# fani-lab/OpeNTF

Hardware: AMD Instinct MI355X
Metric: teams/sec (train) bnn_emb d=128 on DBLP (higher is better)
Workload: dtype f32 (fp16x3 split products, f32 accumulate)

## Files before the change

### opentf_amd/csrc/ntf_engine.hip

```cpp
#include "../../include/opentf_amd.h"
#include "ntf_kernels.h"
#include "ntf_fused.h"
#include "ntf_head.h"

#include <algorithm>
#include <cmath>
#include <cstdio>
#include <cstdlib>
#include <cstring>
#include <string>
#include <vector>

using namespace ntf;

static thread_local std::string g_create_error;

struct LayerInfo {
    int in = 0, out = 0;
    int64_t off[4] = {0, 0, 0, 0};
    int64_t nw() const { return (int64_t)in * out; }
};

enum Fam { F_GATHER = 0, F_GEMM_HIDDEN, F_FLIPOUT_OPERAND, F_OUT_FWD, F_LOSS, F_OUT_BWD_DW, F_OUT_BWD_DA, F_BIAS_GRAD,
           F_FLIPOUT_FINAL, F_KL, F_ADAM, F_SAMPLER, F_INFER, F_OUT_FUSED_FWD, F_OUT_FUSED_DW, F_OUT_FUSED_AUX, F_MULTIHOT, F_COUNT };
// ... 46 lines not shown
    float *partial = nullptr, *row_fix = nullptr, *d_loss = nullptr, *ent_mc = nullptr, *ent_mean = nullptr;
    float *dh_slab = nullptr;
    char* fws = nullptr;
    char* fws_set[2] = {nullptr, nullptr};
    int head_prefetch = 1;
    struct { bool valid = false; uint64_t step = 0; const int64_t* rows = nullptr; int B = 0; int ub = -1; } hp;
    const int64_t* hp_next_rows = nullptr; int hp_next_B = 0;
    const int64_t* hp_next_host = nullptr;
    bool hidden_adam_done = false;
    int64_t hp_used = 0;
    float* gemm_slab = nullptr;
    double* d_kl = nullptr; double* d_acc = nullptr; int64_t* d_acc_steps = nullptr;
    int fwd_kernel = -1;
    int lean = 1;
    int dw_ksplit = 0;
    int32_t* d_range = nullptr;
    int64_t range_fallbacks_host = 0;
    float* tk_vals = nullptr; int32_t* tk_idx = nullptr; int64_t tk_cap = 0;
    std::vector<float*> inj_eps_w, inj_eps_b, inj_s_in, inj_s_out;
    uint64_t seed = 0, step = 0;
    int maxhid = 0;
    int timing = 0;
    std::vector<TimeRec> recs;
    std::vector<hipEvent_t> pool;
    double fam_ms[F_COUNT] = {0}; int64_t fam_calls[F_COUNT] = {0};
    int last_global_B = 0; int last_B = 0; float last_dz_packed_scale = 0.f;
    bool adam_in_dw = false;
    int f32_copy_merged = 1;
    uint64_t f32_copy_step = 0;
    int merge_bias = 1;
// ... 107 lines not shown
    if (cfg->mfma < 0 || cfg->mfma > NTF_MFMA_FP16X3) { g_create_error = "bad mfma"; return NTF_EINVAL; }
    if (cfg->input_mode == NTF_INPUT_MULTIHOT && cfg->n_layers < 2) { g_create_error = "multi-hot input needs a hidden layer (src/mdl/fnn.py:17-19)"; return NTF_EINVAL; }
    int ndev = 0;
    if (hipGetDeviceCount(&ndev) != hipSuccess || ndev < 1) { g_create_error = "no HIP device: the engine has no CPU fallback"; return NTF_EHIP; }
    if (cfg->device < 0 || cfg->device >= ndev) { g_create_error = "device ordinal out of range"; return NTF_EINVAL; }
    if (hipSetDevice(cfg->device) != hipSuccess) { g_create_error = "hipSetDevice failed"; return NTF_EHIP; }
    ntf_engine* e = new ntf_engine();
    e->cfg = *cfg;
    e->L = cfg->n_layers;
    e->lr = cfg->lr;
    e->seed = cfg->seed;
    if (const char* fk = getenv("NTF_FWD_KERNEL")) {
        e->fwd_kernel = atoi(fk);
        if (e->fwd_kernel != 0 && e->fwd_kernel != 5) { g_create_error = "NTF_FWD_KERNEL: 5 (k_out_fwd_h3p, the default) or 0 (k_out_fwd_b6); the forms 1-4 of rounds 2-3 are retired"; delete e; return NTF_EINVAL; }
    }
    if (const char* ks = getenv("NTF_DW_KSPLIT")) e->dw_ksplit = atoi(ks);
    if (const char* ln = getenv("NTF_LEAN")) e->lean = atoi(ln);
    if (const char* hp = getenv("NTF_HEAD_PREFETCH")) e->head_prefetch = atoi(hp);
    if (const char* pf = getenv("NTF_PREFETCH")) e->prefetch = atoi(pf);
    if (const char* hd = getenv("NTF_HEAD")) e->head = atoi(hd);
    if (const char* mb = getenv("NTF_MERGE_BIAS")) e->merge_bias = atoi(mb);
    if (const char* sw = getenv("NTF_L0_SWEEP")) e->l0_sweep = atoi(sw);
    if (const char* fp = getenv("NTF_FNN_PIPE")) e->fnn_pipe = atoi(fp);
    if (const char* mh = getenv("NTF_MH_HEAD")) e->mh_head = atoi(mh);
    if (const char* ek = getenv("NTF_EVAL_KERNEL")) e->eval_kernel = atoi(ek);
    if (const char* nf = getenv("NTF_INFER_F32")) e->infer_f32 = atoi(nf);
    if (const char* fc = getenv("NTF_F32_COPY_MERGED")) e->f32_copy_merged = atoi(fc);
    if (const char* eh = getenv("NTF_EP_HEAD_PREFETCH")) e->ep_head_prefetch = atoi(eh);
    if (const char* dr = getenv("NTF_DP_RANGES")) e->dp_ranges = atoi(dr);
    if (const char* ds = getenv("NTF_DP_SIDE_BWD")) e->dp_side_bwd = atoi(ds);
    if (const char* sb = getenv("NTF_SIDE_BWD")) e->side_bwd = atoi(sb);
// ... 812 lines not shown
        if (side && l == e->L - 2) e->st = e->st3;
        const float* in = e->act[l];
        float* gW = e->G + li.off[NTF_P_WEIGHT]; float* gb = e->G + li.off[NTF_P_BIAS];
        float* gRW = e->cfg.bayesian ? e->G + li.off[NTF_P_RHO_WEIGHT] : nullptr;
        float* gRb = e->cfg.bayesian ? e->G + li.off[NTF_P_RHO_BIAS] : nullptr;
        SignSpec sin_, sout_;
        if (e->cfg.bayesian) { sin_ = sign_spec(e, c, l, T_S_IN, li.in); sout_ = sign_spec(e, c, l, T_S_OUT, li.out); }
        if (last && fused) {
            FusedDw f;
            f.B = B; f.H = li.in; f.M = M; f.bayes = e->cfg.bayesian;
            f.dzT = e->dZout; f.h = in; f.g_mu = gW; f.g_rho = gRW; f.g_b = gb; f.g_bp = gRb; f.ws = e->fws;
            f.mu = e->P + li.off[NTF_P_WEIGHT];
            f.s_out = sout_; f.s_out_inj = e->cfg.bayesian && (sout_.inj != nullptr || sin_.inj != nullptr);
            f.split = e->cfg.mfma != NTF_MFMA_F32 && split_products(e);
            f.a_scale = dz_scale16(e, c.global_B); f.h_scale = kH16Scale; f.rflag = range_ptr(e);
            f.dz_packed = f.split && li.in == 128 && e->pl_mu != nullptr;
            e->last_dz_packed_scale = f.dz_packed ? f.a_scale : 0.f;
            if (f.dz_packed && !c.defer_dw && !(c.fuse_adam && e->cfg.fuse_adam == 2)) {
                const int tiles = (M + fused_dw_tile() - 1) / fused_dw_tile(), nib = fused_ldb(B) / 32;
                int ks = e->dw_ksplit > 0 ? e->dw_ksplit : (tiles <= 128 ? std::min({256 / tiles, 8, std::max(1, nib / 4)}) : 1);
                while (ks > 1 && fused_dw_part_floats(M, li.in, ks) > (int64_t)e->cfg.max_batch * M) --ks;
                if (ks > 1) { f.ksplit = ks; f.part = e->Zout; }
            }
            if (e->cfg.bayesian) { f.rho = e->P + li.off[NTF_P_RHO_WEIGHT]; f.wp = e->Wp[l]; f.klw = kl_share / ((float)out_nw * (float)c.global_B); f.cur_eps = normal_spec(e, c, l, T_EPS_W); }
            if (c.defer_dw) {
                const int tile = fused_dw_tile(), total = (M + tile - 1) / tile;
                e->pend = f; e->pend_valid = true; e->pend_chunks = (total + 255) / 256;
                if (e->cfg.bayesian) { e->pend_eps_b = normal_spec(e, c, l, T_EPS_B); e->pend_klw_b = kl_share / ((float)out_nb * (float)c.global_B); }
                continue;
            }
// ... 54 lines not shown
                    if (gRW) HIPCHK(e, hipMemsetAsync(gRW, 0, (size_t)li.nw() * 4, e->st));
                }
                e->g0_clean = false; e->pre0_step = ~0ull;
                if (l0_sweep_now) HIPCHK(e, hipMemsetAsync(e->l0_touched, 0, (size_t)li.in, e->st));
                launch_multihot_bwd(e->st, c.rows_dev, B, li.in, li.out, e->s_indptr, e->s_indices, dZ, sin_, sout_, gW, gRW, l0_sweep_now ? e->l0_touched : nullptr);
            } else {
                Scope t(e, last ? F_OUT_BWD_DW : F_GEMM_HIDDEN);
                GemmArgs g;
                g.M = li.out; g.N = li.in; g.K = B;
                g.A = dZ; g.sam = 1; g.sak = li.out;
                g.B = in; g.sbk = li.in; g.sbn = 1;
                g.C = gW; g.ldc = li.in;
                const int wtiles = ((li.out + 63) / 64) * ((li.in + 63) / 64);
                if (wtiles < 64 && B >= 256) { g.ksplit = std::max(1, std::min({B >= 2048 ? 64 : 16, B / 64, (int)(kGemmSlabFloats / ((int64_t)li.out * li.in))})); g.slab = e->gemm_slab; }
                if (g.ksplit <= 1) { g.ksplit = 1; g.slab = nullptr; }
                launch_gemm(e->st, g);
                if (e->cfg.bayesian) { g.sa = sout_; g.sa_t = 1; g.sb = sin_; g.sb_t = 0; g.C = gRW; launch_gemm(e->st, g); }
            }
            if (l > 0) {
                Scope t(e, last ? F_OUT_BWD_DA : F_GEMM_HIDDEN);
                float* dA = e->dAct[l & 1];
                GemmArgs g;
                g.M = B; g.N = li.in; g.K = li.out;
                g.A = dZ; g.sam = li.out; g.sak = 1;
                g.B = e->P + li.off[NTF_P_WEIGHT]; g.sbk = li.in; g.sbn = 1;
                g.C = dA; g.ldc = li.in;
                g.mask = e->act[l]; g.ldmask = li.in;
                const int tiles = ((B + 63) / 64) * ((li.in + 63) / 64);
                int ks = 1;
                if (li.out >= 4096) ks = std::max(1, std::min({64, 1024 / tiles, (int)(kGemmSlabFloats / ((int64_t)B * li.in))}));
                g.ksplit = ks; g.slab = e->gemm_slab;
                launch_gemm(e->st, g);
// ... 683 lines not shown
```

### opentf_amd/csrc/ntf_fused.h

```cpp
#pragma once
#include "ntf_kernels.h"

namespace ntf {

struct FusedOut {
    int B = 0, H = 0, M = 0, bayes = 0, train = 0;
    const float* h = nullptr;
    const float *mu = nullptr, *mu_b = nullptr;
    const float *wp = nullptr, *bp = nullptr;
    SignSpec s_in, s_out;
    float tnw = 1.f, tpw = 1.f, inv_B = 1.f;
    float* dzT = nullptr;
    float* dh_slab = nullptr;
    float* dh = nullptr;
    const float* h_mask = nullptr;
    float* loss_partial = nullptr;
    void* ws = nullptr;
    const int64_t* rows = nullptr; const int64_t* m_indptr = nullptr; const int32_t* m_indices = nullptr;
    const int64_t* neg = nullptr; int ns = 0; float* row_fix = nullptr;
    int c_lo = 0;
    int split = 0; uint16_t* mu_pl = nullptr; uint16_t* wp_pl = nullptr;
    float w_scale = 1.f, h_scale = 1.f, dz_scale = 1.f;
    int wide = 5;
    int eval_kernel = 1;
// ... 8 lines not shown

struct FusedDw {
    int B = 0, H = 0, M = 0, bayes = 0;
    const float* dzT = nullptr; const float* h = nullptr;
    const float *mu = nullptr, *rho = nullptr, *wp = nullptr;
    float *g_mu = nullptr, *g_rho = nullptr, *g_b = nullptr, *g_bp = nullptr;
    float klw = 0.f;
    void* ws = nullptr;
    SignSpec s_out; int s_out_inj = 0;
    int adam = 0;
    int split = 0;
    float a_scale = 1.f, h_scale = 1.f;
    int wg_begin = 0, wg_count = 0;
    int* rflag = nullptr;
    int dz_packed = 0;
    int ksplit = 1; float* part = nullptr;
    float *w_mu = nullptr, *w_rho = nullptr, *m_mu = nullptr, *v_mu = nullptr, *m_rho = nullptr, *v_rho = nullptr;
    float lr_over_bc1 = 0.f, b1 = 0.9f, b2 = 0.999f, eps = 1e-8f, bc2_sqrt = 1.f;
    NormalSpec cur_eps;
    int lean = 0;
    int produce = 0; NormalSpec nx_eps; float* nx_wp = nullptr; uint16_t *nx_pl_wp = nullptr, *nx_pl_mu = nullptr; float nx_pscale = 1.f; double nx_klw = 0.0;
    double* nx_kl = nullptr; int* nx_rflag = nullptr;
};

bool fused_supported(int H);
int fused_loss_slots(int M);
int64_t fused_dh_slab_floats(int B, int H, int M);
size_t fused_workspace_bytes(int B, int H, int M);
struct FusedWsPtrs { float *hz, *hs; uint32_t* sinbits; uint16_t* hb; uint32_t* sinT; int Bpad; };
FusedWsPtrs fused_ws_ptrs(void* ws, int B, int H, int M);
// ... 12 lines not shown
```

### opentf_amd/csrc/ntf_fused_dw.hip

```cpp
#include "ntf_fused_common.h"

namespace ntf {

struct DwArgs {
    int B, M, Bpad;
    const float *__restrict__ dzT, *__restrict__ h, *__restrict__ hs, *__restrict__ mu, *__restrict__ rho;
    const float* wp;
    const uint32_t* sbits; int nCB; uint32_t so_k0, so_k1; int so_inj;
    float *__restrict__ g_mu, *__restrict__ g_rho, *__restrict__ g_b, *__restrict__ g_bp;
    float klw;
    float *__restrict__ w_mu, *__restrict__ w_rho, *__restrict__ m_mu, *__restrict__ v_mu, *__restrict__ m_rho, *__restrict__ v_rho;
    float lr_over_bc1, b1, b2, eps, bc2_sqrt;
    int wg_begin;
    int* rflag; int rmode;
    const uint32_t* sT;
    const uint32_t* sinT;
    const uint16_t* hb;
    float a_scale, unscale;
    int ksplit; float* part; int64_t slab; int part_row0;
    unsigned long long* stamps;
    int ntile, stagger;
    NormalSpec cur_eps; int lean;
    int produce; NormalSpec nx_eps; float* nx_wp; uint16_t *nx_pl_wp, *nx_pl_mu; float nx_pscale; double nx_klw; double* nx_kl; int* nx_rflag;
};

__device__ __forceinline__ float adam_update(float p, float g, float& m, float& v, float lr_over_bc1, float b1, float b2, float eps, float bc2_sqrt) {
    adam_step(p, g, m, v, lr_over_bc1, b1, b2, eps, __builtin_amdgcn_rcpf(bc2_sqrt));
    return p;
}

__device__ __forceinline__ uint32_t transpose32(uint32_t a, int il) {
    uint32_t m = 0x0000FFFFu;
#pragma unroll
    for (int j = 16; j != 0; j >>= 1) {
        const uint32_t pv = (uint32_t)__shfl_xor((int)a, j, 64);
// ... 502 lines not shown
#define DWQ_PPG 3
#endif
constexpr int QW = 4;
constexpr int QTC = 32 * QW;
template <bool BAYES, bool ADAM, bool STAMP = false, bool SPLIT = false>
__global__ __launch_bounds__(64 * QW, 2) void k_out_dw_q(DwArgs p) {
    extern __shared__ __attribute__((aligned(16))) char smem[];
    constexpr int H = 128, NJT = 4;
    constexpr int TA = QTC * 32 * 4;
    constexpr int PLANE = H * 64;
    constexpr int TB = 2 * PLANE;
    constexpr int SRC_TB = (BAYES ? 2 : 1) * TB;
    constexpr int TW = BAYES ? 1024 : 0;
    constexpr int STAGE = TA + TB + TW;
    typedef _Float16 h2_t __attribute__((ext_vector_type(2)));
    const int tid = threadIdx.x, lane = tid & 63, wave = tid >> 6, il = lane & 31, half = lane >> 5;
    if (p.rmode == 1 && __builtin_nontemporal_load(p.rflag) != 0) return;
    const int ntile_s = SPLIT ? (int)gridDim.x / p.ksplit : 0;
    const int ksi = SPLIT ? (int)blockIdx.x / ntile_s : 0;
    const int c0 = (p.wg_begin + (SPLIT ? (int)blockIdx.x % ntile_s : (int)blockIdx.x)) * QTC;
    const int crow = wave * 32 + il, c = c0 + crow;
    const int nib = p.Bpad / 32;
    const int ib0 = SPLIT ? (int)((int64_t)ksi * nib / p.ksplit) : 0, ib1 = SPLIT ? (int)((int64_t)(ksi + 1) * nib / p.ksplit) : nib;
    const uint32_t smem_base = lds_addr(smem);
    const int wave_u = __builtin_amdgcn_readfirstlane(wave);
    const char* hb = reinterpret_cast<const char*>(p.hb);
    unsigned long long st_t[4] = {0, 0, 0, 0};
    if (STAMP) st_t[0] = __builtin_amdgcn_s_memrealtime();
    uint32_t lds_base = 0u;
    if (STAMP || (p.stagger > 0 && (int)blockIdx.x < p.ntile)) asm volatile("s_getreg_b32 %0, hwreg(HW_REG_LDS_ALLOC, 0, 8)" : "=s"(lds_base));
    if (p.stagger > 0 && (int)blockIdx.x < p.ntile) {
        if (lds_base != 0u) {
            const uint64_t t0 = __builtin_amdgcn_s_memrealtime();
            while (__builtin_amdgcn_s_memrealtime() - t0 < (uint64_t)p.stagger) __builtin_amdgcn_s_sleep(64);
        }
    }

    const h2_t ones = {(_Float16)1.0f, (_Float16)1.0f};
    constexpr int NA = TA / 1024 / QW, NB = TB / 1024 / QW;
    const float* dz_tile = p.dzT + (int64_t)(c0 >> 8) * nib * 8192 + ((c0 & 255) << 5);
    const uint32_t* sw_src = BAYES ? (half == 0 ? p.sT + (int64_t)(c0 >> 8) * nib * 256 + (c0 & 255) + il * 4 : p.sinT + il * 4) : nullptr;
    const int sw_step = half == 0 ? 256 : 128;
    auto stage_piece = [&](int ib, int buf, int n) {
        const uint32_t sb = smem_base + buf * STAGE;
        if (n < NA) {
            const int inst = wave_u * NA + n;
            const int row = inst * 8 + (lane >> 3), pch = lane & 7;
            const int q = pch ^ ((row >> 1) & 7);
            glds16(dz_tile + (int64_t)ib * 8192 + row * 32 + 4 * q, sb + inst * 1024);
        } else {
            const char* src = hb + (size_t)ib * SRC_TB;
            const int inst = wave_u * NB + (n - NA);
            const int pos = inst * 1024 + lane * 16;
            const int j = (pos % PLANE) >> 6, cd = (pos >> 4) & 3;
            glds16(src + (pos & ~63) + 16 * (cd ^ ((j >> 2) & 3)), sb + TA + inst * 1024);
            if (BAYES && n == NA + NB - 1) glds16(sw_src + (int64_t)ib * sw_step, sb + TA + TB);
        }
    };
    float nx_kl = 0.f, nx_amax = 0.f;
    unsigned long long st_c[3] = {0, 0, 0}, c_prev = 0;
    auto cyc = [&]() -> unsigned long long {
        unsigned long long t;
        __builtin_amdgcn_sched_barrier(0);
        asm volatile("s_memtime %0\n\ts_waitcnt lgkmcnt(0)" : "=s"(t) :: "memory");
        __builtin_amdgcn_sched_barrier(0);
        return t;
    };
#pragma unroll
    for (int n = 0; n < NA + NB; ++n) stage_piece(ib0, 0, n);
    f32x16 acc1[NJT], acc2[NJT];
#pragma unroll
    for (int j = 0; j < NJT; ++j)
#pragma unroll
        for (int r = 0; r < 16; ++r) { acc1[j][r] = 0.f; acc2[j][r] = 0.f; }
    float sum1 = 0.f, sum2 = 0.f;
    const int shl0 = 12 - 4 * half, shl1 = 4 - 4 * half;
    asm volatile("s_waitcnt vmcnt(0)" ::: "memory");
    __syncthreads();
    auto k_block = [&](int ib, auto more_c) {
        constexpr bool MORE = decltype(more_c)::value;
        const int buf = (ib - ib0) & 1;
        const char* sA = smem + buf * STAGE;
        const char* sB = sA + TA;
        uint32_t word = 0u;
        u32x4 iw = {0u, 0u, 0u, 0u};
        if (BAYES) { word = *reinterpret_cast<const uint32_t*>(sA + TA + TB + crow * 4); iw = *reinterpret_cast<const u32x4*>(sA + TA + TB + 512 + il * 16); }
        constexpr int NG = 2 * NJT;
        const char* bbase = sB + il * 64;
        const int swz = (il >> 2) & 3;
        auto load_b = [&](int g, u32x4 (&dst)[2]) {
            const int ks = g / NJT, jt = g % NJT;
            const char* bp = bbase + jt * 2048 + 16 * ((2 * ks + half) ^ swz);
#pragma unroll
// ... 18 lines not shown
                    as[ks][0][q] = s1; as[ks][1][q] = s2;
                    sum2 = __builtin_amdgcn_fdot2(__builtin_bit_cast(h2_t, s1), ones, sum2, false);
                    sum2 = __builtin_amdgcn_fdot2(__builtin_bit_cast(h2_t, s2), ones, sum2, false);
                }
            }
        };
        constexpr int BR = DWQ_BRING;
        u32x4 bq[BR][2], bs[2];
#pragma unroll
        for (int g = 0; g < BR - 1; ++g) load_b(g, bq[g]);
        prep_a(0);
        int piece = 0;
        auto dma = [&]() {
            if (MORE) {
#pragma unroll
                for (int q = 0; q < DWQ_PPG; ++q) { if (piece < NA + NB) stage_piece(ib + 1, buf ^ 1, piece); ++piece; }
            }
        };
#pragma unroll
        for (int g = 0; g < NG; ++g) {
            if (g + BR - 1 < NG) load_b(g + BR - 1, bq[(g + BR - 1) % BR]);
            asm volatile("" ::: "memory");
            const int ks = g / NJT, jt = g % NJT;
            acc1[jt] = mfma3h(a[ks], bq[g % BR], acc1[jt]);
            dma();
            if (BAYES) {
                const uint32_t v = iw[jt] << (ks ? shl1 : shl0);
#pragma unroll
                for (int q = 0; q < 4; ++q) {
                    const uint32_t m = (v << q) & 0x80008000u;
                    bs[0][q] = bq[g % BR][0][q] ^ m; bs[1][q] = bq[g % BR][1][q] ^ m;
                }
                acc2[jt] = mfma3h(as[ks], bs, acc2[jt]);
                dma();
            }
            if (g == 0) prep_a(1);
        }
        if (STAMP) { st_c[0] += cyc() - c_prev; c_prev = cyc(); }
        asm volatile("s_waitcnt vmcnt(0)" ::: "memory");
        if (STAMP) { st_c[1] += cyc() - c_prev; c_prev = cyc(); }
        __syncthreads();
        if (STAMP) { st_c[2] += cyc() - c_prev; c_prev = cyc(); }
    };
    if (STAMP) { st_t[1] = __builtin_amdgcn_s_memrealtime(); c_prev = cyc(); }
    if (DWQ_PRIO) __builtin_amdgcn_s_setprio(DWQ_PRIO);
    for (int ib = ib0; ib < ib1 - 1; ++ib) k_block(ib, std::true_type{});
    k_block(ib1 - 1, std::false_type{});
    if (DWQ_PRIO) __builtin_amdgcn_s_setprio(0);
    if (STAMP) st_t[2] = __builtin_amdgcn_s_memrealtime();
    sum1 += __shfl_xor(sum1, 32, 64);
    sum2 += __shfl_xor(sum2, 32, 64);
    const float inv_a = 1.f / p.a_scale;
    if constexpr (SPLIT) {
        if (half == 0 && c < p.M) {
            float* pb = p.part + (int64_t)p.ksplit * 2 * p.slab; const int64_t Mp = p.slab / 128; const int cl = c - p.part_row0;
            pb[(int64_t)(ksi * 2) * Mp + cl] = sum1 * inv_a; if (BAYES) pb[(int64_t)(ksi * 2 + 1) * Mp + cl] = sum2 * inv_a;
        }
#pragma unroll
        for (int r = 0; r < 16; ++r) {
            const int cr = c0 + wave * 32 + rowmap(r, half);
            if (cr >= p.M) continue;
            const int64_t il0 = (int64_t)(cr - p.part_row0) * H + NJT * il;
            float s1[NJT], s2[NJT];
#pragma unroll
            for (int jt = 0; jt < NJT; ++jt) { s1[jt] = acc1[jt][r] * p.unscale; s2[jt] = acc2[jt][r] * p.unscale; }
            st_vec<NJT>(p.part + (int64_t)(ksi * 2) * p.slab + il0, s1);
            if (BAYES) st_vec<NJT>(p.part + (int64_t)(ksi * 2 + 1) * p.slab + il0, s2);
        }
        return;
    }
    if (half == 0 && c < p.M) { p.g_b[c] = sum1 * inv_a; if (BAYES) p.g_bp[c] = sum2 * inv_a; }

    constexpr int PD = DW_EPI_PD;
    DwOps<NJT> ops[PD + 1];
    auto row_idx = [&](int r, int64_t& idx0) -> bool {
        const int cr = c0 + wave * 32 + rowmap(r, half);
        idx0 = (int64_t)cr * H + NJT * il;
        return cr < p.M;
    };
    static_for<0, PD>([&](auto rc) { constexpr int r = decltype(rc)::value; int64_t idx0; if (row_idx(r, idx0)) dw_ops_load<BAYES, ADAM, NJT>(p, idx0, ops[r % (PD + 1)]); });
    static_for<0, 16>([&](auto rc) {
        constexpr int r = decltype(rc)::value;
        if constexpr (r + PD < 16) { int64_t idn; if (row_idx(r + PD, idn)) dw_ops_load<BAYES, ADAM, NJT>(p, idn, ops[(r + PD) % (PD + 1)]); }
        int64_t idx0;
        if (row_idx(r, idx0)) {
            float s1[NJT], s2[NJT];
#pragma unroll
            for (int jt = 0; jt < NJT; ++jt) { s1[jt] = acc1[jt][r] * p.unscale; s2[jt] = acc2[jt][r] * p.unscale; }
            dw_finish_ops<BAYES, ADAM, NJT>(p, idx0, s1, s2, ops[r % (PD + 1)], nx_kl, nx_amax);
        }
    });
    if (STAMP && p.stamps && lane == 0) {
        asm volatile("s_waitcnt vmcnt(0)" ::: "memory");
        st_t[3] = __builtin_amdgcn_s_memrealtime();
        uint32_t hw_id, xcc;
        asm volatile("s_getreg_b32 %0, hwreg(HW_REG_HW_ID)" : "=s"(hw_id));
        asm volatile("s_getreg_b32 %0, hwreg(HW_REG_XCC_ID)" : "=s"(xcc));
        unsigned long long* o = p.stamps + ((int64_t)blockIdx.x * QW + wave) * 10;
        o[0] = st_t[0]; o[1] = st_t[1]; o[2] = st_t[2]; o[3] = st_t[3]; o[4] = ((unsigned long long)xcc << 32) | hw_id; o[5] = lds_base;
        o[6] = st_c[0]; o[7] = st_c[1]; o[8] = st_c[2]; o[9] = 0;
    }
    if (ADAM && p.produce) dw_produce_finish<BAYES>(p, nx_kl, nx_amax, reinterpret_cast<double*>(smem + 2 * STAGE), QW);
}

void launch_fused_out_dw(hipStream_t st, const FusedDw& f) {
    const Geom g = geom(f.B, f.M);
    const WsLayout w = ws_layout(f.B, f.H, f.M);
    char* ws = static_cast<char*>(f.ws);
    DwArgs a;
    a.B = f.B; a.M = f.M; a.Bpad = g.Bpad; a.dzT = f.dzT; a.h = reinterpret_cast<const float*>(ws + w.hz); a.hs = reinterpret_cast<const float*>(ws + w.hs);
    a.mu = f.mu; a.rho = f.rho; a.wp = f.wp; a.sbits = reinterpret_cast<const uint32_t*>(ws + w.sbits); a.nCB = g.nCB;
    a.so_k0 = f.s_out.k0; a.so_k1 = f.s_out.k1; a.so_inj = f.s_out_inj;
    a.g_mu = f.g_mu; a.g_rho = f.g_rho; a.g_b = f.g_b; a.g_bp = f.g_bp; a.klw = f.klw;
    a.w_mu = f.w_mu; a.w_rho = f.w_rho; a.m_mu = f.m_mu; a.v_mu = f.v_mu; a.m_rho = f.m_rho; a.v_rho = f.v_rho;
    a.lr_over_bc1 = f.lr_over_bc1; a.b1 = f.b1; a.b2 = f.b2; a.eps = f.eps; a.bc2_sqrt = f.bc2_sqrt;
    const int total = (f.M + DW_TC - 1) / DW_TC;
    const int grid = f.wg_count > 0 ? std::min(f.wg_count, total - f.wg_begin) : total;
    a.wg_begin = f.wg_count > 0 ? f.wg_begin : 0;
    if (grid <= 0) return;
    a.hb = reinterpret_cast<const uint16_t*>(ws + w.hb);
    a.rflag = f.rflag; a.rmode = 0;
    a.produce = (f.produce && f.adam && f.H == 128) ? 1 : 0;
    a.cur_eps = f.cur_eps; a.lean = (a.produce && f.lean) ? 1 : 0;
    a.nx_eps = f.nx_eps; a.nx_wp = f.nx_wp; a.nx_pl_wp = f.nx_pl_wp; a.nx_pl_mu = f.nx_pl_mu; a.nx_pscale = f.nx_pscale; a.nx_klw = f.nx_klw; a.nx_kl = f.nx_kl; a.nx_rflag = f.nx_rflag;
    a.ntile = 0; a.stagger = 0; a.stamps = nullptr;
    const bool guard = f.split && f.rflag != nullptr;
    a.sT = reinterpret_cast<const uint32_t*>(ws + w.sbitsT);
    a.ksplit = 1; a.part = nullptr; a.slab = 0; a.part_row0 = 0;
    if (f.H == 256) {
        const size_t lds = 2 * ((size_t)DW_TC * 32 * 4 + (size_t)(f.bayes ? 2 : 1) * 32 * 4 * 128);
#define NTF_DWH(BY, AD) do { auto kf = k_out_dw_h2<BY, AD>; set_max_lds(reinterpret_cast<const void*>(kf), (int)lds);              \
        hipLaunchKernelGGL(kf, dim3(grid, 2), dim3(64 * DW_WAVES), lds, st, a); } while (0)
        if (f.bayes) { if (f.adam) NTF_DWH(true, true); else NTF_DWH(true, false); } else { if (f.adam) NTF_DWH(false, true); else NTF_DWH(false, false); }
#undef NTF_DWH
        return;
    }
    if (f.split && f.dz_packed) {
        a.a_scale = f.a_scale; a.unscale = 1.f / (f.a_scale * f.h_scale); a.rmode = guard ? 1 : 0;
        const int ks = (f.ksplit > 1 && f.part) ? std::min(f.ksplit, std::max(1, g.Bpad / 32)) : 1;
        if (ks > 1) {
// ... 14 lines not shown
            if (!guard) return;
            a.rmode = 2; a.ksplit = 1; a.wg_begin = wg256; a.part_row0 = 0;
            goto exact_f32;
        }
        {
            a.sinT = reinterpret_cast<const uint32_t*>(ws + w.sinT);
            const int total_q = (f.M + QTC - 1) / QTC, qb = f.wg_count > 0 ? 2 * f.wg_begin : 0;
            const int qgrid = f.wg_count > 0 ? std::min(2 * f.wg_count, total_q - qb) : total_q;
            const int wg256 = a.wg_begin;
            a.wg_begin = qb;
            static int n_cu = 0;
            if (!n_cu) { int dev = 0; hipGetDevice(&dev); hipDeviceGetAttribute(&n_cu, hipDeviceAttributeMultiprocessorCount, dev); if (n_cu <= 0) n_cu = 256; }
            static const int stagger_q = getenv("NTF_DW_STAGGER") ? atoi(getenv("NTF_DW_STAGGER")) : -1;
            const int nib = g.Bpad / 32;
            a.ntile = 2 * n_cu;
            a.stagger = (f.adam && qgrid > n_cu) ? (stagger_q >= 0 ? stagger_q : (nib * 140 + 4500) / 2) : 0;
            const size_t ldsq = 2 * ((size_t)QTC * 128 + 2 * 128 * 64 + (f.bayes ? 1024 : 0)) + 64;
#define NTF_DWQ(BY, AD) do { auto kf = k_out_dw_q<BY, AD>;                                                                     \
            set_max_lds(reinterpret_cast<const void*>(kf), (int)ldsq);     \
            hipLaunchKernelGGL(kf, dim3(qgrid), dim3(64 * QW), ldsq, st, a); } while (0)
#ifdef NTF_DIAG
            static const char* stamp_file = getenv("NTF_DW_STAMP_FILE");
#else
            static const char* stamp_file = nullptr;
#endif
            if (stamp_file && f.bayes && f.adam) {
                static unsigned long long* d_st = nullptr; static int n_launch = 0;
                if (!d_st) hipMalloc(&d_st, (size_t)qgrid * QW * 10 * 8);
                a.stamps = d_st;
                auto kf = k_out_dw_q<true, true, true>;
                set_max_lds(reinterpret_cast<const void*>(kf), (int)ldsq);
                hipLaunchKernelGGL(kf, dim3(qgrid), dim3(64 * QW), ldsq, st, a);
                if (++n_launch == 30) {
                    std::vector<unsigned long long> hst((size_t)qgrid * QW * 10);
                    hipStreamSynchronize(st); hipMemcpy(hst.data(), d_st, hst.size() * 8, hipMemcpyDeviceToHost);
                    if (FILE* fp = fopen(stamp_file, "wb")) { fwrite(hst.data(), 8, hst.size(), fp); fclose(fp); }
                }
            }
            else if (f.bayes) { if (f.adam) NTF_DWQ(true, true); else NTF_DWQ(true, false); } else { if (f.adam) NTF_DWQ(false, true); else NTF_DWQ(false, false); }
#undef NTF_DWQ
            if (!guard) return;
            a.rmode = 2; a.wg_begin = wg256; a.ntile = 0; a.stagger = 0;
            goto exact_f32;
        }
    }
    if (f.split) {
        a.rmode = guard ? 1 : 0;
// ... 43 lines not shown
```

### opentf_amd/csrc/ntf_kernels.h

```cpp
#pragma once
#include <hip/hip_runtime.h>
#include <stdint.h>

namespace ntf {

constexpr float kLeakySlope = 0.01f;

struct SignSpec {
    const float* inj = nullptr;
    int64_t ld = 0;
    uint32_t k0 = 0, k1 = 0;
    int enabled = 0;
};

struct NormalSpec {
    const float* inj = nullptr;
    uint32_t k0 = 0, k1 = 0, tag = 0, step = 0;
    int64_t qbase = 0;
};

struct GemmArgs {
    int M = 0, N = 0, K = 0;
    const float* A = nullptr; int64_t sam = 0, sak = 0;
    const float* B = nullptr; int64_t sbk = 0, sbn = 0;
    SignSpec sa; int sa_t = 0;
    SignSpec sb; int sb_t = 0;
    float* C = nullptr; int64_t ldc = 0;
    float* Act = nullptr; int64_t ldact = 0;
    const float* bias = nullptr;
    SignSpec sc;
    const float* mask = nullptr; int64_t ldmask = 0;
    int accumulate = 0;
    int ksplit = 1;
    float* slab = nullptr;
    float alpha = 1.0f;
};

void launch_gemm(hipStream_t st, const GemmArgs& a);

void launch_gather_meanpool(hipStream_t st, const int64_t* indptr, const int32_t* indices, const float* table,
                            const int64_t* rows, int64_t n, int d, int mean, float* out);
void launch_gather_dense_rows(hipStream_t st, const float* X, int d, const int64_t* rows, int64_t n, float* out);
void launch_multihot_fwd(hipStream_t st, const int64_t* rows, int B, int S, int H, const int64_t* indptr, const int32_t* indices,
                         const float* W, const float* b, const float* Wp , const float* bp, SignSpec sin, SignSpec sout, float* act);
void launch_multihot_bwd(hipStream_t st, const int64_t* rows, int B, int S, int H, const int64_t* indptr, const int32_t* indices,
                         const float* dZ, SignSpec sin, SignSpec sout, float* gW , float* gWp , uint8_t* touched = nullptr);

struct PerturbChain { double* kl_out2 = nullptr; int* mu_flag_out = nullptr; const int* raise_if = nullptr; };
void launch_flipout_perturb(hipStream_t st, const float* rho, const float* mu, int64_t n, NormalSpec eps, float* out, double w, double* kl_out,
                            uint16_t* planes_w = nullptr, uint16_t* planes_mu = nullptr, const float* pmu = nullptr, int H = 0,
                            float pscale = 1.f,
                            int* rflag = nullptr ,
                            const int* only_if = nullptr ,
// ... 55 lines not shown
```

### opentf_amd/csrc/ntf_kernels.hip

```cpp
#include "ntf_kernels.h"
#include <cstdlib>
#include "ntf_device.h"
#include <algorithm>
#include <cstdint>

namespace ntf {

constexpr int GBM = 64, GBN = 64, GBK = 32, GLD = GBK + 1;

__global__ __launch_bounds__(256) void k_gemm(GemmArgs a) {
    __shared__ float As[GBM * GLD];
    __shared__ float Bs[GBN * GLD];
    const int tid = threadIdx.x, lane = tid & 63, wave = tid >> 6;
    const int m0 = blockIdx.y * GBM, n0 = blockIdx.x * GBN;
    int kper = (a.K + a.ksplit - 1) / a.ksplit;
    kper = (kper + GBK - 1) / GBK * GBK;
    const int kbeg = blockIdx.z * kper;
    const int kend = min(a.K, kbeg + kper);
    const bool a_kc = (a.sak == 1), b_nc = (a.sbn == 1);
    f32x16 acc;
#pragma unroll
    for (int i = 0; i < 16; ++i) acc[i] = 0.f;
    const int wm = wave >> 1, wn = wave & 1;

// ... 63 lines not shown
    if (e >= mn) return;
    float s = 0.f;
    for (int z = 0; z < ks; ++z) s += slab[(int64_t)z * mn + e];
    const int64_t o = (e / N) * ldc + (e % N);
    C[o] = accumulate ? C[o] + s : s;
}

void launch_gemm(hipStream_t st, const GemmArgs& a) {
    if (a.M <= 0 || a.N <= 0) return;
    dim3 grid((a.N + GBN - 1) / GBN, (a.M + GBM - 1) / GBM, a.ksplit > 1 ? a.ksplit : 1);
    hipLaunchKernelGGL(k_gemm, grid, dim3(256), 0, st, a);
    if (a.ksplit > 1) {
        const int64_t mn = (int64_t)a.M * a.N;
        hipLaunchKernelGGL(k_gemm_reduce, dim3((unsigned)((mn + 255) / 256)), dim3(256), 0, st, a.slab, a.ksplit, mn, a.N, a.C, a.ldc, a.accumulate);
    }
}

template <int G>
__global__ __launch_bounds__(256) void k_gather_pool(const int64_t* __restrict__ indptr, const int32_t* __restrict__ indices,
                                                     const float* __restrict__ table, const int64_t* __restrict__ rows,
                                                     int64_t n, int d, int mean, int vec, float* __restrict__ out) {
    constexpr int TPW = 64 / G;
    const int lane = threadIdx.x & 63, sub = lane / G, sl = lane % G;
    const int64_t wave_global = ((int64_t)blockIdx.x * blockDim.x + threadIdx.x) >> 6;
    const int64_t t = wave_global * TPW + sub;
    const bool live = t < n;
    const int64_t team = live ? (rows ? rows[t] : t) : 0;
    const int64_t beg = live ? indptr[team] : 0, end = live ? indptr[team + 1] : 0;
    const int nnz = (int)(end - beg);
    const int nchunk = (d + 4 * G - 1) / (4 * G);
// ... 904 lines not shown
```

Measured before the change: 676,400.

## Add persistent tile walk to output dW kernel and fused hidden-layer dW kernel

The output-layer dW kernel (k_out_dw_q) can now run as a persistent grid capped at a slot count. Each workgroup walks several column tiles and prefetches the next tile's operands while it runs the current tile's epilogue. A new k_hidden_dw kernel computes the hidden-layer weight gradient and its flipout counterpart in one launch, reducing the k-split partials in LDS instead of going through the slab-plus-reduce GEMM path. This removes launch and reduction-kernel overhead for small hidden layers. The costs are higher register pressure in the persistent loop and a less tiled, f32-MFMA hidden kernel that reads operands straight from global memory.

```diff
diff --git a/opentf_amd/csrc/ntf_engine.hip b/opentf_amd/csrc/ntf_engine.hip
--- a/opentf_amd/csrc/ntf_engine.hip
+++ b/opentf_amd/csrc/ntf_engine.hip
@@ -84,6 +84,9 @@
     int fwd_kernel = -1;
     int lean = 1;
     int dw_ksplit = 0;
+    int dw_persist = 1;
+    int dw_slots = 0;
+    int hidden_dw = 1;
     int32_t* d_range = nullptr;
     int64_t range_fallbacks_host = 0;
     float* tk_vals = nullptr; int32_t* tk_idx = nullptr; int64_t tk_cap = 0;
@@ -221,7 +224,13 @@
         e->fwd_kernel = atoi(fk);
         if (e->fwd_kernel != 0 && e->fwd_kernel != 5) { g_create_error = "NTF_FWD_KERNEL: 5 (k_out_fwd_h3p, the default) or 0 (k_out_fwd_b6); the forms 1-4 of rounds 2-3 are retired"; delete e; return NTF_EINVAL; }
     }
+    if (const char* dk = getenv("NTF_DW_KERNEL")) {
+        if (atoi(dk) != 1) { g_create_error = "NTF_DW_KERNEL: 1 (k_out_dw_q, the default); round 3's one-workgroup-per-CU form 0 was retired in round 6"; delete e; return NTF_EINVAL; }
+    }
     if (const char* ks = getenv("NTF_DW_KSPLIT")) e->dw_ksplit = atoi(ks);
+    if (const char* dp = getenv("NTF_DW_PERSIST")) e->dw_persist = atoi(dp) != 0;
+    if (const char* sl = getenv("NTF_DW_SLOTS")) e->dw_slots = std::max(0, atoi(sl));
+    if (const char* hd = getenv("NTF_HIDDEN_DW")) e->hidden_dw = atoi(hd) != 0;
     if (const char* ln = getenv("NTF_LEAN")) e->lean = atoi(ln);
     if (const char* hp = getenv("NTF_HEAD_PREFETCH")) e->head_prefetch = atoi(hp);
     if (const char* pf = getenv("NTF_PREFETCH")) e->prefetch = atoi(pf);
@@ -1064,6 +1073,7 @@
             f.s_out = sout_; f.s_out_inj = e->cfg.bayesian && (sout_.inj != nullptr || sin_.inj != nullptr);
             f.split = e->cfg.mfma != NTF_MFMA_F32 && split_products(e);
             f.a_scale = dz_scale16(e, c.global_B); f.h_scale = kH16Scale; f.rflag = range_ptr(e);
+            f.persist = e->dw_persist; f.slots = e->dw_slots;
             f.dz_packed = f.split && li.in == 128 && e->pl_mu != nullptr;
             e->last_dz_packed_scale = f.dz_packed ? f.a_scale : 0.f;
             if (f.dz_packed && !c.defer_dw && !(c.fuse_adam && e->cfg.fuse_adam == 2)) {
@@ -1148,8 +1158,14 @@
                 const int wtiles = ((li.out + 63) / 64) * ((li.in + 63) / 64);
                 if (wtiles < 64 && B >= 256) { g.ksplit = std::max(1, std::min({B >= 2048 ? 64 : 16, B / 64, (int)(kGemmSlabFloats / ((int64_t)li.out * li.in))})); g.slab = e->gemm_slab; }
                 if (g.ksplit <= 1) { g.ksplit = 1; g.slab = nullptr; }
+                if (e->hidden_dw && hidden_dw_supported(li.in, li.out)) {
+                    HiddenDw hd; hd.B = B; hd.D = li.in; hd.H = li.out; hd.ksplit = g.ksplit; hd.dz = dZ; hd.x = in; hd.g_w = gW;
+                    if (e->cfg.bayesian) { hd.g_wp = gRW; hd.s_out = sout_; hd.s_in = sin_; }
+                    launch_hidden_dw(e->st, hd);
+                } else {
                 launch_gemm(e->st, g);
                 if (e->cfg.bayesian) { g.sa = sout_; g.sa_t = 1; g.sb = sin_; g.sb_t = 0; g.C = gRW; launch_gemm(e->st, g); }
+                }
             }
             if (l > 0) {
                 Scope t(e, last ? F_OUT_BWD_DA : F_GEMM_HIDDEN);
diff --git a/opentf_amd/csrc/ntf_fused.h b/opentf_amd/csrc/ntf_fused.h
--- a/opentf_amd/csrc/ntf_fused.h
+++ b/opentf_amd/csrc/ntf_fused.h
@@ -46,6 +46,7 @@
     int wg_begin = 0, wg_count = 0;
     int* rflag = nullptr;
     int dz_packed = 0;
+    int persist = 1, slots = 0;
     int ksplit = 1; float* part = nullptr;
     float *w_mu = nullptr, *w_rho = nullptr, *m_mu = nullptr, *v_mu = nullptr, *m_rho = nullptr, *v_rho = nullptr;
     float lr_over_bc1 = 0.f, b1 = 0.9f, b2 = 0.999f, eps = 1e-8f, bc2_sqrt = 1.f;
diff --git a/opentf_amd/csrc/ntf_fused_dw.hip b/opentf_amd/csrc/ntf_fused_dw.hip
--- a/opentf_amd/csrc/ntf_fused_dw.hip
+++ b/opentf_amd/csrc/ntf_fused_dw.hip
@@ -19,6 +19,7 @@
     float a_scale, unscale;
     int ksplit; float* part; int64_t slab; int part_row0;
     unsigned long long* stamps;
+    int nwalk;
     int ntile, stagger;
     NormalSpec cur_eps; int lean;
     int produce; NormalSpec nx_eps; float* nx_wp; uint16_t *nx_pl_wp, *nx_pl_mu; float nx_pscale; double nx_klw; double* nx_kl; int* nx_rflag;
@@ -551,16 +552,17 @@
     constexpr int TW = BAYES ? 1024 : 0;
     constexpr int STAGE = TA + TB + TW;
     typedef _Float16 h2_t __attribute__((ext_vector_type(2)));
-    const int tid = threadIdx.x, lane = tid & 63, wave = tid >> 6, il = lane & 31, half = lane >> 5;
+    int tid = threadIdx.x, lane = tid & 63, wave = tid >> 6, il = lane & 31, half = lane >> 5;
     if (p.rmode == 1 && __builtin_nontemporal_load(p.rflag) != 0) return;
     const int ntile_s = SPLIT ? (int)gridDim.x / p.ksplit : 0;
     const int ksi = SPLIT ? (int)blockIdx.x / ntile_s : 0;
-    const int c0 = (p.wg_begin + (SPLIT ? (int)blockIdx.x % ntile_s : (int)blockIdx.x)) * QTC;
-    const int crow = wave * 32 + il, c = c0 + crow;
+    int t = SPLIT ? (int)blockIdx.x % ntile_s : (int)blockIdx.x;
+    int c0 = (p.wg_begin + t) * QTC;
+    int crow = wave * 32 + il;
     const int nib = p.Bpad / 32;
     const int ib0 = SPLIT ? (int)((int64_t)ksi * nib / p.ksplit) : 0, ib1 = SPLIT ? (int)((int64_t)(ksi + 1) * nib / p.ksplit) : nib;
     const uint32_t smem_base = lds_addr(smem);
-    const int wave_u = __builtin_amdgcn_readfirstlane(wave);
+    int wave_u = __builtin_amdgcn_readfirstlane(wave);
     const char* hb = reinterpret_cast<const char*>(p.hb);
     unsigned long long st_t[4] = {0, 0, 0, 0};
     if (STAMP) st_t[0] = __builtin_amdgcn_s_memrealtime();
@@ -575,10 +577,12 @@
 
     const h2_t ones = {(_Float16)1.0f, (_Float16)1.0f};
     constexpr int NA = TA / 1024 / QW, NB = TB / 1024 / QW;
-    const float* dz_tile = p.dzT + (int64_t)(c0 >> 8) * nib * 8192 + ((c0 & 255) << 5);
-    const uint32_t* sw_src = BAYES ? (half == 0 ? p.sT + (int64_t)(c0 >> 8) * nib * 256 + (c0 & 255) + il * 4 : p.sinT + il * 4) : nullptr;
-    const int sw_step = half == 0 ? 256 : 128;
-    auto stage_piece = [&](int ib, int buf, int n) {
+    auto dz_of = [&](int c0_) -> const float* { return p.dzT + (int64_t)(c0_ >> 8) * nib * 8192 + ((c0_ & 255) << 5); };
+    auto sw_of = [&](int c0_) -> const uint32_t* { return BAYES ? (half == 0 ? p.sT + (int64_t)(c0_ >> 8) * nib * 256 + (c0_ & 255) + il * 4 : p.sinT + il * 4) : nullptr; };
+    const float* dz_tile = dz_of(c0);
+    const uint32_t* sw_src = sw_of(c0);
+    int sw_step = half == 0 ? 256 : 128;
+    auto stage_piece = [&](const float* dz_tile, const uint32_t* sw_src, int ib, int buf, int n) {
         const uint32_t sb = smem_base + buf * STAGE;
         if (n < NA) {
             const int inst = wave_u * NA + n;
@@ -594,7 +598,6 @@
             if (BAYES && n == NA + NB - 1) glds16(sw_src + (int64_t)ib * sw_step, sb + TA + TB);
         }
     };
-    float nx_kl = 0.f, nx_amax = 0.f;
     unsigned long long st_c[3] = {0, 0, 0}, c_prev = 0;
     auto cyc = [&]() -> unsigned long long {
         unsigned long long t;
@@ -604,16 +607,10 @@
         return t;
     };
 #pragma unroll
-    for (int n = 0; n < NA + NB; ++n) stage_piece(ib0, 0, n);
+    for (int n = 0; n < NA + NB; ++n) stage_piece(dz_tile, sw_src, ib0, 0, n);
     f32x16 acc1[NJT], acc2[NJT];
-#pragma unroll
-    for (int j = 0; j < NJT; ++j)
-#pragma unroll
-        for (int r = 0; r < 16; ++r) { acc1[j][r] = 0.f; acc2[j][r] = 0.f; }
-    float sum1 = 0.f, sum2 = 0.f;
-    const int shl0 = 12 - 4 * half, shl1 = 4 - 4 * half;
-    asm volatile("s_waitcnt vmcnt(0)" ::: "memory");
-    __syncthreads();
+    float sum1, sum2;
+    int shl0 = 12 - 4 * half, shl1 = 4 - 4 * half;
     auto k_block = [&](int ib, auto more_c) {
         constexpr bool MORE = decltype(more_c)::value;
         const int buf = (ib - ib0) & 1;
@@ -662,7 +659,7 @@
         auto dma = [&]() {
             if (MORE) {
 #pragma unroll
-                for (int q = 0; q < DWQ_PPG; ++q) { if (piece < NA + NB) stage_piece(ib + 1, buf ^ 1, piece); ++piece; }
+                for (int q = 0; q < DWQ_PPG; ++q) { if (piece < NA + NB) stage_piece(dz_tile, sw_src, ib + 1, buf ^ 1, piece); ++piece; }
             }
         };
 #pragma unroll
@@ -690,12 +687,36 @@
         __syncthreads();
         if (STAMP) { st_c[2] += cyc() - c_prev; c_prev = cyc(); }
     };
+    for (;;) {
+    if (!SPLIT) {
+        asm volatile("" : "+v"(tid));
+        lane = tid & 63; wave = tid >> 6; il = lane & 31; half = lane >> 5; crow = wave * 32 + il; wave_u = __builtin_amdgcn_readfirstlane(wave);
+        sw_step = half == 0 ? 256 : 128; shl0 = 12 - 4 * half; shl1 = 4 - 4 * half;
+        dz_tile = dz_of(c0); sw_src = sw_of(c0);
+    }
+    float nx_kl = 0.f, nx_amax = 0.f;
+    const int c = c0 + crow;
+#pragma unroll
+    for (int j = 0; j < NJT; ++j)
+#pragma unroll
+        for (int r = 0; r < 16; ++r) { acc1[j][r] = 0.f; acc2[j][r] = 0.f; }
+    sum1 = 0.f; sum2 = 0.f;
+    asm volatile("s_waitcnt vmcnt(0)" ::: "memory");
+    __syncthreads();
     if (STAMP) { st_t[1] = __builtin_amdgcn_s_memrealtime(); c_prev = cyc(); }
     if (DWQ_PRIO) __builtin_amdgcn_s_setprio(DWQ_PRIO);
     for (int ib = ib0; ib < ib1 - 1; ++ib) k_block(ib, std::true_type{});
     k_block(ib1 - 1, std::false_type{});
     if (DWQ_PRIO) __builtin_amdgcn_s_setprio(0);
     if (STAMP) st_t[2] = __builtin_amdgcn_s_memrealtime();
+    const int t_next = SPLIT ? 0 : t + (int)gridDim.x;
+    const bool more_tiles = !SPLIT && t_next < p.nwalk;
+    const int c0_next = (p.wg_begin + t_next) * QTC;
+    if (more_tiles) {
+        const float* dzn = dz_of(c0_next); const uint32_t* swn = sw_of(c0_next);
+#pragma unroll
+        for (int n = 0; n < NA + NB; ++n) stage_piece(dzn, swn, ib0, 0, n);
+    }
     sum1 += __shfl_xor(sum1, 32, 64);
     sum2 += __shfl_xor(sum2, 32, 64);
     const float inv_a = 1.f / p.a_scale;
@@ -720,22 +741,24 @@
     if (half == 0 && c < p.M) { p.g_b[c] = sum1 * inv_a; if (BAYES) p.g_bp[c] = sum2 * inv_a; }
 
     constexpr int PD = DW_EPI_PD;
-    DwOps<NJT> ops[PD + 1];
+    DwArgs pe = p;
+    asm volatile("" : "+s"(pe.cur_eps.k0), "+s"(pe.cur_eps.k1), "+s"(pe.nx_eps.k0), "+s"(pe.nx_eps.k1));
+    DwOps<NJT> ops[PD + 1] = {};
     auto row_idx = [&](int r, int64_t& idx0) -> bool {
         const int cr = c0 + wave * 32 + rowmap(r, half);
         idx0 = (int64_t)cr * H + NJT * il;
         return cr < p.M;
     };
-    static_for<0, PD>([&](auto rc) { constexpr int r = decltype(rc)::value; int64_t idx0; if (row_idx(r, idx0)) dw_ops_load<BAYES, ADAM, NJT>(p, idx0, ops[r % (PD + 1)]); });
+    static_for<0, PD>([&](auto rc) { constexpr int r = decltype(rc)::value; int64_t idx0; if (row_idx(r, idx0)) dw_ops_load<BAYES, ADAM, NJT>(pe, idx0, ops[r % (PD + 1)]); });
     static_for<0, 16>([&](auto rc) {
         constexpr int r = decltype(rc)::value;
-        if constexpr (r + PD < 16) { int64_t idn; if (row_idx(r + PD, idn)) dw_ops_load<BAYES, ADAM, NJT>(p, idn, ops[(r + PD) % (PD + 1)]); }
+        if constexpr (r + PD < 16) { int64_t idn; if (row_idx(r + PD, idn)) dw_ops_load<BAYES, ADAM, NJT>(pe, idn, ops[(r + PD) % (PD + 1)]); }
         int64_t idx0;
         if (row_idx(r, idx0)) {
             float s1[NJT], s2[NJT];
 #pragma unroll
             for (int jt = 0; jt < NJT; ++jt) { s1[jt] = acc1[jt][r] * p.unscale; s2[jt] = acc2[jt][r] * p.unscale; }
-            dw_finish_ops<BAYES, ADAM, NJT>(p, idx0, s1, s2, ops[r % (PD + 1)], nx_kl, nx_amax);
+            dw_finish_ops<BAYES, ADAM, NJT>(pe, idx0, s1, s2, ops[r % (PD + 1)], nx_kl, nx_amax);
         }
     });
     if (STAMP && p.stamps && lane == 0) {
@@ -744,11 +767,15 @@
         uint32_t hw_id, xcc;
         asm volatile("s_getreg_b32 %0, hwreg(HW_REG_HW_ID)" : "=s"(hw_id));
         asm volatile("s_getreg_b32 %0, hwreg(HW_REG_XCC_ID)" : "=s"(xcc));
-        unsigned long long* o = p.stamps + ((int64_t)blockIdx.x * QW + wave) * 10;
+        unsigned long long* o = p.stamps + ((int64_t)t * QW + wave) * 10;
         o[0] = st_t[0]; o[1] = st_t[1]; o[2] = st_t[2]; o[3] = st_t[3]; o[4] = ((unsigned long long)xcc << 32) | hw_id; o[5] = lds_base;
         o[6] = st_c[0]; o[7] = st_c[1]; o[8] = st_c[2]; o[9] = 0;
     }
     if (ADAM && p.produce) dw_produce_finish<BAYES>(p, nx_kl, nx_amax, reinterpret_cast<double*>(smem + 2 * STAGE), QW);
+    if (!more_tiles) break;
+    t = t_next; c0 = c0_next;
+    if (STAMP) { st_t[0] = __builtin_amdgcn_s_memrealtime(); st_c[0] = st_c[1] = st_c[2] = 0; }
+    }
 }
 
 void launch_fused_out_dw(hipStream_t st, const FusedDw& f) {
@@ -771,7 +798,7 @@
     a.produce = (f.produce && f.adam && f.H == 128) ? 1 : 0;
     a.cur_eps = f.cur_eps; a.lean = (a.produce && f.lean) ? 1 : 0;
     a.nx_eps = f.nx_eps; a.nx_wp = f.nx_wp; a.nx_pl_wp = f.nx_pl_wp; a.nx_pl_mu = f.nx_pl_mu; a.nx_pscale = f.nx_pscale; a.nx_klw = f.nx_klw; a.nx_kl = f.nx_kl; a.nx_rflag = f.nx_rflag;
-    a.ntile = 0; a.stagger = 0; a.stamps = nullptr;
+    a.ntile = 0; a.nwalk = 0; a.stagger = 0; a.stamps = nullptr;
     const bool guard = f.split && f.rflag != nullptr;
     a.sT = reinterpret_cast<const uint32_t*>(ws + w.sbitsT);
     a.ksplit = 1; a.part = nullptr; a.slab = 0; a.part_row0 = 0;
@@ -816,11 +843,14 @@
             static const int stagger_q = getenv("NTF_DW_STAGGER") ? atoi(getenv("NTF_DW_STAGGER")) : -1;
             const int nib = g.Bpad / 32;
             a.ntile = 2 * n_cu;
+            const int slots = std::max(1, std::min(f.slots > 0 ? f.slots : 2 * n_cu, 2 * n_cu));
+            a.nwalk = qgrid;
+            const int wgrid = f.persist ? std::min(qgrid, slots) : qgrid;
             a.stagger = (f.adam && qgrid > n_cu) ? (stagger_q >= 0 ? stagger_q : (nib * 140 + 4500) / 2) : 0;
             const size_t ldsq = 2 * ((size_t)QTC * 128 + 2 * 128 * 64 + (f.bayes ? 1024 : 0)) + 64;
 #define NTF_DWQ(BY, AD) do { auto kf = k_out_dw_q<BY, AD>;                                                                     \
             set_max_lds(reinterpret_cast<const void*>(kf), (int)ldsq);     \
-            hipLaunchKernelGGL(kf, dim3(qgrid), dim3(64 * QW), ldsq, st, a); } while (0)
+            hipLaunchKernelGGL(kf, dim3(wgrid), dim3(64 * QW), ldsq, st, a); } while (0)
 #ifdef NTF_DIAG
             static const char* stamp_file = getenv("NTF_DW_STAMP_FILE");
 #else
@@ -832,7 +862,7 @@
                 a.stamps = d_st;
                 auto kf = k_out_dw_q<true, true, true>;
                 set_max_lds(reinterpret_cast<const void*>(kf), (int)ldsq);
-                hipLaunchKernelGGL(kf, dim3(qgrid), dim3(64 * QW), ldsq, st, a);
+                hipLaunchKernelGGL(kf, dim3(wgrid), dim3(64 * QW), ldsq, st, a);
                 if (++n_launch == 30) {
                     std::vector<unsigned long long> hst((size_t)qgrid * QW * 10);
                     hipStreamSynchronize(st); hipMemcpy(hst.data(), d_st, hst.size() * 8, hipMemcpyDeviceToHost);
diff --git a/opentf_amd/csrc/ntf_kernels.h b/opentf_amd/csrc/ntf_kernels.h
--- a/opentf_amd/csrc/ntf_kernels.h
+++ b/opentf_amd/csrc/ntf_kernels.h
@@ -37,6 +37,16 @@
 };
 
 void launch_gemm(hipStream_t st, const GemmArgs& a);
+
+struct HiddenDw {
+    int B = 0, D = 0, H = 0, ksplit = 1;
+    const float* dz = nullptr;
+    const float* x = nullptr;
+    float* g_w = nullptr; float* g_wp = nullptr;
+    SignSpec s_out, s_in;
+};
+bool hidden_dw_supported(int D, int H);
+void launch_hidden_dw(hipStream_t st, const HiddenDw& a);
 
 void launch_gather_meanpool(hipStream_t st, const int64_t* indptr, const int32_t* indices, const float* table,
                             const int64_t* rows, int64_t n, int d, int mean, float* out);
diff --git a/opentf_amd/csrc/ntf_kernels.hip b/opentf_amd/csrc/ntf_kernels.hip
--- a/opentf_amd/csrc/ntf_kernels.hip
+++ b/opentf_amd/csrc/ntf_kernels.hip
@@ -101,6 +101,69 @@
         const int64_t mn = (int64_t)a.M * a.N;
         hipLaunchKernelGGL(k_gemm_reduce, dim3((unsigned)((mn + 255) / 256)), dim3(256), 0, st, a.slab, a.ksplit, mn, a.N, a.C, a.ldc, a.accumulate);
     }
+}
+
+constexpr int HDW_WAVES = 16;
+__global__ __launch_bounds__(64 * HDW_WAVES) void k_hidden_dw(HiddenDw a) {
+    __shared__ float part[HDW_WAVES][1024];
+    const int tid = threadIdx.x, lane = tid & 63, wave = tid >> 6, il = lane & 31, kh = lane >> 5;
+    const int m0 = blockIdx.y * 32, n0 = blockIdx.x * 32;
+    const bool flip = blockIdx.z != 0;
+    float* __restrict__ C = flip ? a.g_wp : a.g_w;
+    int kper = (a.B + a.ksplit - 1) / a.ksplit;
+    kper = (kper + GBK - 1) / GBK * GBK;
+    const int gm = m0 + il, gn = n0 + il;
+    float run = 0.f;
+    for (int z0 = 0; z0 < a.ksplit; z0 += HDW_WAVES) {
+        const int z = z0 + wave;
+        if (z < a.ksplit) {
+            const int kbeg = z * kper, kend = min(a.B, kbeg + kper);
+            f32x16 acc;
+#pragma unroll
+            for (int i = 0; i < 16; ++i) acc[i] = 0.f;
+            for (int k0 = kbeg; k0 < kend; k0 += GBK) {
+                float ra[GBK / 2], rb[GBK / 2];
+#pragma unroll
+                for (int kk = 0; kk < GBK / 2; ++kk) {
+                    const int gk = k0 + 2 * kk + kh;
+                    float v = 0.f, w = 0.f;
+                    if (gk < kend) {
+                        if (gm < a.H) { v = a.dz[(int64_t)gk * a.H + gm]; if (flip) v *= sign_at(a.s_out, gk, gm); }
+                        if (gn < a.D) { w = a.x[(int64_t)gk * a.D + gn]; if (flip) w *= sign_at(a.s_in, gk, gn); }
+                    }
+                    ra[kk] = v; rb[kk] = w;
+                }
+#pragma unroll
+                for (int kk = 0; kk < GBK / 2; ++kk) acc = __builtin_amdgcn_mfma_f32_32x32x2f32(ra[kk], rb[kk], acc, 0, 0, 0);
+            }
+            if (a.ksplit == 1) {
+                if (gn < a.D) {
+#pragma unroll
+                    for (int r = 0; r < 16; ++r) {
+                        const int row = m0 + (r & 3) + 8 * (r >> 2) + 4 * kh;
+                        if (row < a.H) C[(int64_t)row * a.D + gn] = acc[r] * 1.0f + 0.f;
+                    }
+                }
+            } else {
+#pragma unroll
+                for (int r = 0; r < 16; ++r) part[wave][r * 64 + lane] = acc[r] * 1.0f + 0.f;
+            }
+        }
+        if (a.ksplit == 1) return;
+        __syncthreads();
+        const int nz = min(HDW_WAVES, a.ksplit - z0);
+        for (int w = 0; w < nz; ++w) run += part[w][tid];
+        __syncthreads();
+    }
+    const int r = tid >> 6;
+    const int row = m0 + (r & 3) + 8 * (r >> 2) + 4 * kh;
+    if (row < a.H && gn < a.D) C[(int64_t)row * a.D + gn] = run;
+}
+
+bool hidden_dw_supported(int D, int H) { return D >= 1 && D <= 256 && (H == 32 || H == 64 || H == 128); }
+void launch_hidden_dw(hipStream_t st, const HiddenDw& a) {
+    if (a.B <= 0) return;
+    hipLaunchKernelGGL(k_hidden_dw, dim3((a.D + 31) / 32, a.H / 32, a.g_wp ? 2 : 1), dim3(64 * HDW_WAVES), 0, st, a);
 }
 
 template <int G>
```

Result: no change. 675,900 (-0.1%).
